# faverogian/diffusion-classifier

Hardware: AMD Instinct MI355X
Metric: images classified/sec (node), CIFAR-10 10-class x 50-step ELBO scoring (higher is better)
Workload: dtype bf16; 1 GPU; cifar10-unet-10x50; classes=10, trials=50, forwards_per_image=500, input=uniform [-1,1], parallelism=single

## Files before the change

diffusion-classifier_amd/csrc/conv3_halo.h:

```cpp
#pragma once
#include <stdlib.h>
#include "igemm_epilogue.h"

typedef const __attribute__((address_space(1))) void* gptr_t;
typedef __attribute__((address_space(3))) void* lptr_t;

struct HaloGeom {
  int ltw, lth, lni;
  int tiles_x, tiles_y;
  int hw, hp, HR, nxl;
  int n_img, H, W;
  float inv_hp, inv_hw;
  int mos, lmc;
  float inv_ch, inv_cw;
  int xbuf;
  int sws;
  int lpt;
};


constexpr int HALO_WST = 128 * 64;

template <int NW> struct HaloCfg {
  static constexpr int NT = NW * 64;
  static constexpr int PIX = NW * 64;
  static constexpr int NXL = NW == 4 ? 6 : 7;
  static constexpr int XBUF = NXL * NT * 16;
  static constexpr int XROWS = NXL * NT / 4;
  static constexpr int WLD = 512 / NT;
  static constexpr int WR = NW == 4 ? 3 : 4;
  static constexpr int GNOFF = 2 * XBUF + WR * HALO_WST;
  static constexpr int GNMAXC = 512;
  static constexpr int TBLOFF = GNOFF + 2 * GNMAXC * 4;
  static constexpr int LDS_MAIN = TBLOFF + 128;
  static constexpr int LDS = LDS_MAIN;
};

__device__ __forceinline__ int swz64(int row) { return (0x78 >> (((row >> 2) & 3) << 1)) & 3; }
__device__ __forceinline__ int lds64_off(int row, int chunk) { return row * 64 + ((chunk ^ swz64(row)) << 4); }


struct HaloQs {
  static constexpr bool on = true;
  int nbase, ltp, n_img, tile_in_img, wm, np, padd;
  __device__ __forceinline__ bool whole() const { return ltp >= 7; }
  __device__ __forceinline__ int parts() const { return np; }
  __device__ __forceinline__ bool operator()(int half, int& n, int& part) const {
    const int p0 = wm * 128 + half * 64;
    n = nbase + (p0 >> ltp);
    part = padd + (ltp >= 7 ? (tile_in_img << (ltp - 7)) + ((p0 & ((1 << ltp) - 1)) >> 7) : tile_in_img);
    return n < n_img;
  }
};

struct HaloLdsBias {
  static constexpr bool on = true, has_rowvec = true;
  const float* p;
  __device__ __forceinline__ void operator()(int k, float (&bs)[8], float (&)[8]) const {
    const f32x4 lo = *reinterpret_cast<const f32x4*>(p + 32 * k), hi = *reinterpret_cast<const f32x4*>(p + 32 * k + 4);
#pragma unroll
    for (int e = 0; e < 4; ++e) { bs[e] = lo[e]; bs[4 + e] = hi[e]; }
  }
};

template <int N> __device__ __forceinline__ void hwait_vmcnt() { asm volatile("s_waitcnt vmcnt(%0)" ::"n"(N) : "memory"); }

template <int V> struct IC { static constexpr int value = V; };
```

diffusion-classifier_amd/csrc/conv3_halo.hip:

```cpp
#include <stdlib.h>
#include "common.h"
#ifdef DC_STAMPS
static __device__ unsigned long long* g_stamps;
extern "C" void dc_debug_set_stamps(unsigned long long* p) { (void)hipMemcpyToSymbol(HIP_SYMBOL(g_stamps), &p, sizeof(p)); }
#define DC_STAMP(k) do { if (threadIdx.x == 0 && g_stamps) g_stamps[blockIdx.x * 8 + (k)] = __builtin_amdgcn_s_memtime(); } while (0)
static __device__ int g_halo_abl;
extern "C" void dc_debug_set_halo_abl(int v) { (void)hipMemcpyToSymbol(HIP_SYMBOL(g_halo_abl), &v, sizeof(v)); }
#define DC_HALO_ABL() __builtin_amdgcn_readfirstlane(g_halo_abl)
#else
#define DC_STAMP(k) do {} while (0)
#define DC_HALO_ABL() 0
#endif
#include "igemm_epilogue.h"
#include "epi_pn.h"

static __device__ unsigned g_pn_timeouts;
static __device__ chunk16 g_zero_page[16];
#include "conv3_halo.h"
DC_CLOCK_DECL(conv3_halo)

template <typename T, int NW, int NTAP = 9, int MODE = 0, bool STG = false, bool PN = false>
__global__ __launch_bounds__(NW * 64, 2) void conv3_halo_kernel(const IgemmArgs a, const HaloGeom g) {
  static_assert(!PN || (MODE == 1 && NW == 4 && !STG) || ((MODE == 0 || MODE == 2) && NW == 8 && STG && NTAP == 9), "producer-side GroupNorm: one-image-per-patch forms, or 8x8 / 4x4 images");
  constexpr bool PNX = PN && NW == 4, PNL = PN && NW == 8;
  static_assert(!STG || NW == 8, "staggered loop: the 8-wave kernel");
  constexpr bool XB = MODE == 1, MOS = MODE == 2;
  using Cfg = HaloCfg<NW>;
  constexpr int EPC = Elem<T>::EPC;
  constexpr int BKE = 4 * EPC;
  constexpr int TM = 8, TN = 4;
  constexpr int NT = Cfg::NT, WLD = Cfg::WLD, WR = Cfg::WR, PD = Cfg::WR - 1;
  extern __shared__ __attribute__((aligned(16))) char smem[];
  char* const Wring = smem + 2 * Cfg::XBUF;

  DC_STAMP(0);
  const int t = threadIdx.x;
  const int lane = t & 63;
  const int wave = __builtin_amdgcn_readfirstlane(t >> 6);
  const int wm = wave >> 1, wn = wave & 1;
  const int lr = lane & 15, lq = lane >> 4;
  int tile_m, tile_n;
  if constexpr (PNX) {
    constexpr int LPH = NTAP == 4 ? 2 : 0;
    const int tnr = a.tiles_n >> LPH;
    const int kq = blockIdx.x >> 3;
    const int grp = ((kq >> (g.lpt + LPH)) << 3) + (blockIdx.x & 7);
    if (grp >= g.n_img * tnr) return;
    const int smp = grp / tnr;
    const int within = kq & ((1 << (g.lpt + LPH)) - 1);
    tile_n = __builtin_amdgcn_readfirstlane((within >> g.lpt) * tnr + grp - smp * tnr);
    tile_m = __builtin_amdgcn_readfirstlane((smp << g.lpt) + (within & ((1 << g.lpt) - 1)));
    asm volatile("" : "+s"(tile_m), "+s"(tile_n));
  } else if constexpr (XB) tile_of_block_scalar(a, tile_m, tile_n);
  else tile_of_block(a, tile_m, tile_n);
  constexpr bool UP4 = NTAP == 4;
  int phase = 0;
  if (UP4) { const int tn = a.tiles_n >> 2; phase = tile_n / tn; tile_n -= phase * tn; }
  const int pa = phase >> 1, pb = phase & 1;
  const int tx = tile_m % g.tiles_x;
  const int ty = (tile_m / g.tiles_x) % g.tiles_y;
  const int ng = tile_m / (g.tiles_x * g.tiles_y);
  const int tw = 1 << g.ltw, th = 1 << g.lth;
  const int HW = g.H * g.W;
  const int HWs = a.upsample ? (g.H >> 1) * (g.W >> 1) : HW;
  const int Ctot = a.C0 + a.C1;
  const int c0chunks = a.C0 / BKE, nchunks = Ctot / BKE;

  constexpr int NXL = Cfg::NXL;
  int pp[NXL];
  const int xlx = t & 3;
  int* const tbl = reinterpret_cast<int*>(smem + Cfg::TBLOFF);
  if (t < (1 << g.lni)) {
    const int n = (ng << g.lni) + t;
    const bool vn = n < g.n_img;
    tbl[4 * t] = vn ? (a.map0 ? a.map0[n] : n) * HWs : -1;
    tbl[4 * t + 1] = (vn && a.src1) ? (a.map1 ? a.map1[n] : n) * HWs : -1;
    tbl[4 * t + 2] = (vn && a.src2) ? (a.map2 ? a.map2[n] : n) * HWs : -1;
  }
  auto piece_code = [&](int i, int* col = nullptr) -> int {
    const int hr = (i * NT + t) >> 2;
    int code = -1;
    if (col) *col = 0;
    if (i < g.nxl && hr < g.HR) {
      if constexpr (MOS) {
        const int hy = (int)(((float)hr + 0.5f) * g.inv_hw), hx = hr - hy * g.hw;
        const int cy = (int)(((float)hy + 0.5f) * g.inv_ch), ry = hy - cy * (th + 1);
        const int cx = (int)(((float)hx + 0.5f) * g.inv_cw), rx = hx - cx * (tw + 1);
        if (col) *col = hx;
        if (ry > 0 && rx > 0) code = (((cy << g.lmc) + cx) << 20) | ((ry - 1) * g.W + rx - 1);
      } else {
        const int img = (int)(((float)hr + 0.5f) * g.inv_hp), r = hr - img * g.hp;
        const int hy = (int)(((float)r + 0.5f) * g.inv_hw), hx = r - hy * g.hw;
        const int iy = ty * th + hy - 1, ix = tx * tw + hx - 1;
        if (col) *col = hx;
        if ((unsigned)iy < (unsigned)g.H && (unsigned)ix < (unsigned)g.W)
          code = (img << 20) | (a.upsample ? (iy >> 1) * (g.W >> 1) + (ix >> 1) : iy * g.W + ix);
      }
    }
    return code;
  };
  constexpr bool SWP = !STG;
#pragma unroll
  for (int i = 0; i < NXL; ++i) {
    int col;
    pp[i] = piece_code(i, &col);
    if constexpr (SWP) { if (pp[i] >= 0) pp[i] |= ((col >> g.sws) & 1) << 30; }
  }
  auto sw_of = [&](int pk) -> int { if constexpr (SWP) return (pk >> 30) & 1; else return 0; };
  constexpr int PKMASK = SWP ? 0x3FFFFFFF : -1;
  float* const brv = reinterpret_cast<float*>(smem + Cfg::GNOFF);
  constexpr bool STAGE_BRV = XB;
  if (STAGE_BRV && t < 128) {
    const int c = tile_n * 128 + t;
    float v = 0.f;
    if (c < a.Cout) {
      if (a.bias) v = a.bias[c];
      if (a.rowvec) v += a.rowvec[(size_t)(a.rowvec_map ? a.rowvec_map[ng] : ng) * a.rowvec_ld + c];
    }
    brv[t] = v;
  }
  if constexpr (PNX) {
    if (t >= 128 && t < 256) {
      const int c = tile_n * 128 + t - 128;
      brv[t] = a.pn_gamma[c];
      brv[t + 128] = a.pn_beta[c];
    }
  }
  __syncthreads();
  const char* zero = reinterpret_cast<const char*>(g_zero_page);
  constexpr bool XROW = STG && !XB;
  auto retarget = [&](int which) {
#pragma unroll
    for (int i = 0; i < NXL; ++i) {
      const int code = piece_code(i);
      int row = -1;
      if (code >= 0) {
        const int b = tbl[4 * (code >> 20) + which];
        if (b >= 0) row = b + (code & 0xFFFFF);
      }
      pp[i] = row;
    }
  };
  if constexpr (XROW) retarget(0);

  const T* xb0 = nullptr; const T* xb1 = nullptr; const T* xb2 = nullptr;
  int wvoff = 0, ldb0 = 0, ldb1 = 0, ldb2 = 0;
  if (XB) {
    ldb0 = a.ld0 * (int)sizeof(T); ldb1 = a.ld1 * (int)sizeof(T); ldb2 = a.ld2 * (int)sizeof(T);
    asm volatile("" : "+s"(ldb0), "+s"(ldb1), "+s"(ldb2));
    const int n = ng;
    const int s0 = __builtin_amdgcn_readfirstlane(a.map0 ? a.map0[n] : n);
    xb0 = reinterpret_cast<const T*>(a.src0) + (size_t)s0 * HWs * a.ld0;
    if (a.src1) { const int s1 = __builtin_amdgcn_readfirstlane(a.map1 ? a.map1[n] : n); xb1 = reinterpret_cast<const T*>(a.src1) + (size_t)s1 * HWs * a.ld1; }
    if (a.src2) { const int s2 = __builtin_amdgcn_readfirstlane(a.map2 ? a.map2[n] : n); xb2 = reinterpret_cast<const T*>(a.src2) + (size_t)s2 * HWs * a.ld2; }
  }
  if (XB || STG) {
    const int wrow0 = t >> 2;
    wvoff = (epi_wrow(wrow0, false) * a.Ktot + ((t & 3) ^ swz64(wrow0)) * EPC) * (int)sizeof(T);
  }
  auto rsrc_of = [](const void* base) { return __builtin_amdgcn_make_buffer_rsrc(const_cast<void*>(base), 0, 0x7fffffff, 0x00020000); };

  auto issue_x = [&](int cc, int i0 = 0, int i1 = 64) {
    const int which = cc >= nchunks ? 2 : (cc >= c0chunks ? 1 : 0);
    if constexpr (XB) {
      int ldb = ldb0, cb = cc;
      const T* xb = xb0;
      if (cc >= nchunks) { ldb = ldb2; cb = cc - nchunks; xb = xb2; }
      else if (cc >= c0chunks) { ldb = ldb1; cb = cc - c0chunks; xb = xb1; }
      const int cofs = cb * 64 + xlx * 16;
      const __amdgpu_buffer_rsrc_t rs = rsrc_of(xb);
      char* xs = smem + (cc & 1) * Cfg::XBUF + wave * 1024;
#pragma unroll
      for (int i = 0; i < NXL; ++i) {
        if (i < i0 || i >= i1) continue;
        int pk = pp[i];
        asm volatile("" : "+v"(pk));
        const int voff = pk < 0 ? -1 : (pk & PKMASK) * ldb + (cofs ^ (sw_of(pk) << 5));
        __builtin_amdgcn_raw_ptr_buffer_load_lds(rs, (lptr_t)(xs + i * (NT * 16)), 16, voff, 0, 0, 0);
      }
      return;
    } else {
    const T* src = reinterpret_cast<const T*>(which == 2 ? a.src2 : (which == 1 ? a.src1 : a.src0));
    const int ld = which == 2 ? a.ld2 : (which == 1 ? a.ld1 : a.ld0);
    const int coff = (which == 2 ? cc - nchunks : (which == 1 ? cc - c0chunks : cc)) * BKE + xlx * EPC;
    char* xs = smem + (cc & 1) * Cfg::XBUF + wave * 1024;
#pragma unroll
    for (int i = 0; i < NXL; ++i) {
      if (i < i0 || i >= i1) continue;
      int pk = pp[i];
      asm volatile("" : "+v"(pk));
      int rowi;
      if constexpr (XROW) rowi = pk;
      else {
        const int base = pk < 0 ? -1 : tbl[4 * ((pk & PKMASK) >> 20) + which];
        rowi = base < 0 ? -1 : base + (pk & 0xFFFFF);
      }
      const size_t e = (size_t)(rowi < 0 ? 0 : rowi) * ld + (coff ^ (sw_of(pk) << 1) * EPC);
      const char* gp = rowi < 0 ? zero : reinterpret_cast<const char*>(src + e);
      __builtin_amdgcn_global_load_lds((gptr_t)gp, (lptr_t)(xs + i * (NT * 16)), 16, 0, 0);
    }
    }
  };
  const int wtile0 = ((UP4 ? phase * (a.tiles_n >> 2) : 0) + tile_n) * 128 * a.Ktot;
  auto issue_w = [&](int cc, int tap, int slot) {
    if constexpr (XB || STG) {
      const int so = (wtile0 + tap * Ctot + cc * BKE) * (int)sizeof(T);
      const __amdgpu_buffer_rsrc_t wrs = rsrc_of(a.W);
#pragma unroll
      for (int i = 0; i < WLD; ++i)
        __builtin_amdgcn_raw_ptr_buffer_load_lds(wrs, (lptr_t)(Wring + slot * HALO_WST + i * (NT * 16) + wave * 1024), 16, wvoff,
                                                 __builtin_amdgcn_readfirstlane(so + i * 64 * a.Ktot * (int)sizeof(T)), 0, 0);
    } else {
      const T* wb = reinterpret_cast<const T*>(a.W) + (size_t)wtile0 + (size_t)tap * Ctot + (size_t)cc * BKE;
      int tt = t;
      asm volatile("" : "+v"(tt));
#pragma unroll
      for (int i = 0; i < WLD; ++i) {
        const int row = (i * NT + tt) >> 2;
        const int wro = epi_wrow(row, false) * a.Ktot + ((tt & 3) ^ swz64(row)) * EPC;
        __builtin_amdgcn_global_load_lds((gptr_t) reinterpret_cast<const char*>(wb + wro),
                                         (lptr_t)(Wring + slot * HALO_WST + i * (NT * 16) + wave * 1024), 16, 0, 0);
      }
    }
  };

  auto issue_w2 = [&](int e, int slot) {
    int tt = t;
    asm volatile("" : "+v"(tt));
#pragma unroll
    for (int i = 0; i < WLD; ++i) {
      const int row = (i * NT + tt) >> 2;
      const T* wp = reinterpret_cast<const T*>(a.W2) + (size_t)(tile_n * 128 + epi_wrow(row, false)) * a.C2 + ((tt & 3) ^ swz64(row)) * EPC + e * BKE;
      __builtin_amdgcn_global_load_lds((gptr_t) reinterpret_cast<const char*>(wp),
                                       (lptr_t)(Wring + slot * HALO_WST + i * (NT * 16) + wave * 1024), 16, 0, 0);
    }
  };
  const int nx = a.src2 ? a.C2 / BKE : 0;

  constexpr int NV = 3;
  int xlv[NV];
  {
    const int xx = lr & ((tw < 16 ? tw : 16) - 1);
    const int rowpart = ((lr >> g.ltw) * g.hw + (lr & (tw - 1))) * 64;
#pragma unroll
    for (int k = 0; k < NV; ++k) xlv[k] = rowpart + ((lq ^ (SWP ? (((xx + k + (UP4 ? pb : 0)) >> g.sws) & 1) << 1 : 0)) << 4);
  }
  int joff[TM];
#pragma unroll
  for (int j = 0; j < TM; ++j) {
    const int p = wm * 128 + j * 16;
    const int img = p >> (g.ltw + g.lth), py = (p >> g.ltw) & (th - 1), px = p & (tw - 1);
    const int o = MOS ? ((img >> g.lmc) * (th + 1) + py) * g.hw + (img & ((1 << g.lmc) - 1)) * (tw + 1) + px : img * g.hp + py * g.hw + px;
    joff[j] = __builtin_amdgcn_readfirstlane(o * 64);
  }
  const int woff0 = lds64_off(wn * 64 + lr, lq);

  f32x4 acc[TN][TM];
#pragma unroll
  for (int i = 0; i < TN; ++i)
#pragma unroll
    for (int j = 0; j < TM; ++j) acc[i][j] = f32x4{0.f, 0.f, 0.f, 0.f};

  auto mma_tap = [&](const char* Wst, const char* Xb, int tapoff, auto kxc) {
    constexpr int kx = decltype(kxc)::value;
    chunk16 wf[TN];
#pragma unroll
    for (int i = 0; i < TN; ++i) wf[i] = *reinterpret_cast<const chunk16*>(Wst + woff0 + i * 1024);
#pragma unroll
    for (int h = 0; h < 2; ++h) {
      chunk16 xf[TM / 2];
#pragma unroll
      for (int j = 0; j < TM / 2; ++j) xf[j] = *reinterpret_cast<const chunk16*>(Xb + (tapoff + joff[h * (TM / 2) + j]) + xlv[MOS ? ((kx + j) & 1) : kx]);
#pragma unroll
      for (int j = 0; j < TM / 2; ++j)
#pragma unroll
        for (int i = 0; i < TN; ++i) acc[i][h * (TM / 2) + j] = Mma<T>::run(wf[i], xf[j], acc[i][h * (TM / 2) + j]);
      if (h == 0) __builtin_amdgcn_sched_barrier(0);
    }
  };

  DC_STAMP(1);
  if constexpr (STG) {
    const bool grpB = wave >= 4;
    const int abl = DC_HALO_ABL();
    int cur_which = 0;
    issue_x(0);
#pragma unroll
    for (int i = 0; i < PD; ++i) issue_w(0, i, i);
    hwait_vmcnt<0>();
    __builtin_amdgcn_s_barrier();
    if (grpB) __builtin_amdgcn_s_barrier();
    DC_CLOCK(0);
    chunk16 wf[TN], xf[TM / 2];
    const uint32_t lds0 = lds_addr_of(smem);
    uint32_t xaddr[TM];
#pragma unroll
    for (int j = 0; j < TM; ++j) xaddr[j] = lds0 + (uint32_t)(joff[j] + xlv[0]);
    const uint32_t waddr = lds_addr_of(Wring) + (uint32_t)woff0;
    for (int cc = 0; cc < nchunks; ++cc) {
      const bool side_next = cc + 1 == nchunks && nx > 0;
      const bool has_next = cc + 1 < nchunks || side_next;
      const int s0 = cc * NTAP;
      const uint32_t xbo = (uint32_t)(cc & 1) * Cfg::XBUF;
      if constexpr (XROW) {
        const int wnext = cc + 1 >= nchunks ? 2 : (cc + 1 >= c0chunks ? 1 : 0);
        if (has_next && wnext != cur_which) { retarget(wnext); cur_which = wnext; }
      }
      auto step = [&](auto tapc) {
        constexpr int tap = decltype(tapc)::value;
        constexpr int ky = UP4 ? (tap >> 1) : tap / 3, kx = UP4 ? (tap & 1) : tap - ky * 3;
        const uint32_t rowo = xbo + (uint32_t)(((ky + pa) * g.hw + pb) * 64);
        const uint32_t wso = (uint32_t)((s0 + tap) % WR) * HALO_WST;
        __builtin_amdgcn_s_barrier();
        __builtin_amdgcn_sched_barrier(0);
        if (!(abl & 2)) {
        wf[0] = ds_read16_async_off<0>(waddr + wso);
        wf[1] = ds_read16_async_off<1024>(waddr + wso);
        wf[2] = ds_read16_async_off<2048>(waddr + wso);
        wf[3] = ds_read16_async_off<3072>(waddr + wso);
#pragma unroll
        for (int j = 0; j < TM / 2; ++j) xf[j] = ds_read16_async_off<kx * 64>(xaddr[j] + rowo);
        }
        constexpr int t2 = tap + PD;
#ifndef DC_STG_W_IN_M
        if (!(abl & 4)) {
        if (t2 < NTAP) issue_w(cc, t2, (s0 + t2) % WR);
        else if (side_next) { if (t2 - NTAP < nx) issue_w2(t2 - NTAP, (s0 + t2) % WR); }
        else if (has_next) issue_w(cc + 1, t2 - NTAP, (s0 + t2) % WR);
        }
#endif
#ifdef DC_STG_WAIT_FIRST
        asm volatile("s_waitcnt lgkmcnt(0)" : "+v"(wf[0]), "+v"(wf[1]), "+v"(wf[2]), "+v"(wf[3]), "+v"(xf[0]), "+v"(xf[1]), "+v"(xf[2]), "+v"(xf[3]));
        __builtin_amdgcn_s_barrier();
#else
        __builtin_amdgcn_s_barrier();
        asm volatile("s_waitcnt lgkmcnt(0)" : "+v"(wf[0]), "+v"(wf[1]), "+v"(wf[2]), "+v"(wf[3]), "+v"(xf[0]), "+v"(xf[1]), "+v"(xf[2]), "+v"(xf[3]));
#endif
        __builtin_amdgcn_sched_barrier(0);
        if (!(abl & 1)) {
#pragma unroll
        for (int i = 0; i < TN; ++i) acc[i][0] = Mma<T>::run(wf[i], xf[0], acc[i][0]);
        }
        __builtin_amdgcn_sched_barrier(0);
#ifdef DC_STG_W_IN_M
        if (!(abl & 4)) {
        if (t2 < NTAP) issue_w(cc, t2, (s0 + t2) % WR);
        else if (side_next) { if (t2 - NTAP < nx) issue_w2(t2 - NTAP, (s0 + t2) % WR); }
        else if (has_next) issue_w(cc + 1, t2 - NTAP, (s0 + t2) % WR);
        }
#endif
        __builtin_amdgcn_sched_barrier(0);
        if (!(abl & 1)) {
#pragma unroll
        for (int j = 1; j < TM / 2; ++j)
#pragma unroll
          for (int i = 0; i < TN; ++i) acc[i][j] = Mma<T>::run(wf[i], xf[j], acc[i][j]);
        }
        __builtin_amdgcn_sched_barrier(0);
        __builtin_amdgcn_s_barrier();
        __builtin_amdgcn_sched_barrier(0);
        if (!(abl & 2)) {
#pragma unroll
        for (int j = 0; j < TM / 2; ++j) xf[j] = ds_read16_async_off<kx * 64>(xaddr[TM / 2 + j] + rowo);
        }
        constexpr int XP_A = UP4 ? (tap == 1 ? NXL : 0) : (tap == 1 ? 2 : (tap >= 2 && tap <= 6 ? 1 : 0));
#ifndef DC_STG_X_IN_M
        constexpr int XP_C = UP4 ? (tap == 0 ? NXL : 0) : (tap == 0 ? 2 : (tap <= 5 ? 1 : 0));
        if (has_next && !(abl & 12)) {
          if constexpr (UP4) { if (tap == 0) issue_x(cc + 1); }
          else if constexpr (tap == 0) issue_x(cc + 1, 0, 2);
          else if constexpr (tap <= 5) issue_x(cc + 1, tap + 1, tap + 2);
        }
        constexpr int XP_B = XP_C + (UP4 ? (tap == 2 ? NXL : 0) : (tap == 2 ? 2 : (tap >= 3 && tap <= 7 ? 1 : 0)));
#else
        constexpr int XP_B = UP4 ? (tap == 2 ? NXL : 0) : (tap == 2 ? 2 : (tap >= 3 && tap <= 7 ? 1 : 0));
#endif
        if (has_next) {
          if (tap == NTAP - 1 && side_next && nx < PD) hwait_vmcnt<0>();
          else hwait_vmcnt<(PD - 1) * WLD + XP_A + XP_B>();
        } else {
          constexpr int left = NTAP - 1 - tap;
          if constexpr (left > 0) hwait_vmcnt<((left - 1) < (PD - 1) ? (left - 1) : (PD - 1)) * WLD>();
        }
#ifdef DC_STG_WAIT_FIRST
        asm volatile("s_waitcnt lgkmcnt(0)" : "+v"(xf[0]), "+v"(xf[1]), "+v"(xf[2]), "+v"(xf[3]));
        __builtin_amdgcn_s_barrier();
#else
        __builtin_amdgcn_s_barrier();
        asm volatile("s_waitcnt lgkmcnt(0)" : "+v"(xf[0]), "+v"(xf[1]), "+v"(xf[2]), "+v"(xf[3]));
#endif
        __builtin_amdgcn_sched_barrier(0);
        if (!(abl & 1)) {
#pragma unroll
        for (int i = 0; i < TN; ++i) acc[i][TM / 2] = Mma<T>::run(wf[i], xf[0], acc[i][TM / 2]);
        }
        __builtin_amdgcn_sched_barrier(0);
#ifdef DC_STG_X_IN_M
        if (has_next && !(abl & 12)) {
          if constexpr (UP4) { if (tap == 0) issue_x(cc + 1); }
          else if constexpr (tap == 0) issue_x(cc + 1, 0, 2);
          else if constexpr (tap <= 5) issue_x(cc + 1, tap + 1, tap + 2);
        }
#endif
        __builtin_amdgcn_sched_barrier(0);
        if (!(abl & 1)) {
#pragma unroll
        for (int j = 1; j < TM / 2; ++j)
#pragma unroll
          for (int i = 0; i < TN; ++i) acc[i][TM / 2 + j] = Mma<T>::run(wf[i], xf[j], acc[i][TM / 2 + j]);
        }
        __builtin_amdgcn_sched_barrier(0);
      };
      step(IC<0>{}); step(IC<1>{}); step(IC<2>{}); step(IC<3>{});
      if constexpr (NTAP == 9) { step(IC<4>{}); step(IC<5>{}); step(IC<6>{}); step(IC<7>{}); step(IC<8>{}); }
    }
    if (!grpB) __builtin_amdgcn_s_barrier();
    DC_CLOCK(1);
  } else {
  issue_x(0);
#pragma unroll
  for (int i = 0; i < PD; ++i) issue_w(0, i, i);
  constexpr int FLYL = (PD - 1) * WLD;
  DC_CLOCK(0);
  for (int cc = 0; cc < nchunks; ++cc) {
    const bool side_next = cc + 1 == nchunks && nx > 0;
    const bool has_next = cc + 1 < nchunks || side_next;
    const int s0 = cc * NTAP;
    const char* Xb = smem + (cc & 1) * Cfg::XBUF;
    auto step = [&](auto tapc) {
      constexpr int tap = decltype(tapc)::value;
      if (has_next) {
        if (tap >= 1 && tap <= PD) hwait_vmcnt<FLYL + NXL>();
        else hwait_vmcnt<FLYL>();
      } else {
        constexpr int left = NTAP - 1 - tap;
        hwait_vmcnt<(left < PD - 1 ? left : PD - 1) * WLD>();
      }
      __builtin_amdgcn_s_barrier();
      constexpr int t2 = tap + PD;
      if (t2 < NTAP) issue_w(cc, t2, (s0 + t2) % WR);
      else if (side_next) { if (t2 - NTAP < nx) issue_w2(t2 - NTAP, (s0 + t2) % WR); }
      else if (has_next) issue_w(cc + 1, t2 - NTAP, (s0 + t2) % WR);
      if (tap == 0 && has_next) issue_x(cc + 1);

      const char* Wst = Wring + ((s0 + tap) % WR) * HALO_WST;
      constexpr int ky = UP4 ? (tap >> 1) : tap / 3, kx = UP4 ? (tap & 1) : tap - ky * 3;
      const int tapoff = ((ky + pa) * g.hw + kx + pb) * 64;
      mma_tap(Wst, Xb, tapoff, IC<kx>{});
    };
    step(IC<0>{}); step(IC<1>{}); step(IC<2>{}); step(IC<3>{});
    if constexpr (NTAP == 9) { step(IC<4>{}); step(IC<5>{}); step(IC<6>{}); step(IC<7>{}); step(IC<8>{}); }
  }

  DC_CLOCK(1);
  }
  constexpr int FLY = (PD - 1) * WLD;
  {
    const int NSm = nchunks * NTAP;
    for (int e = 0; e < nx; ++e) {
      if (e == 0 && nx >= PD) hwait_vmcnt<FLY>();
      else hwait_vmcnt<0>();
      __builtin_amdgcn_s_barrier();
      if (e + PD < nx) issue_w2(e + PD, (NSm + e + PD) % WR);
      if (e + 1 < nx) issue_x(nchunks + e + 1);
      const char* Xb = smem + ((nchunks + e) & 1) * Cfg::XBUF;
      const char* Wst = Wring + ((NSm + e) % WR) * HALO_WST;
      const int tapoff = (g.hw + 1) * 64;
      mma_tap(Wst, Xb, tapoff, IC<1>{});
    }
  }

  DC_STAMP(2);
  const int nw0 = min((ng << g.lni) + ((wm * 128) >> (g.ltw + g.lth)), g.n_img - 1);
  const int nw1 = min((ng << g.lni) + ((wm * 128 + 127) >> (g.ltw + g.lth)), g.n_img - 1);
  HaloQs qsfn;
  qsfn.nbase = ng << g.lni; qsfn.ltp = g.ltw + g.lth; qsfn.n_img = g.n_img; qsfn.tile_in_img = ty * g.tiles_x + tx; qsfn.wm = wm;
  qsfn.np = HW >= 128 ? HW >> 7 : 1;
  qsfn.padd = 0;
  if (UP4) { qsfn.padd = phase * qsfn.np; qsfn.np *= 4; }
  auto rowfn = [&](int j, EpiRow& r) {
    const int p = wm * 128 + j * 16 + lr;
    int n = (ng << g.lni) + (p >> (g.ltw + g.lth));
    r.ok = n < g.n_img;
    n = r.ok ? n : g.n_img - 1;
    const int py = (p >> g.ltw) & (th - 1), px = p & (tw - 1);
    const int rem = (ty * th + py) * g.W + tx * tw + px;
    r.samp = n;
    r.o = UP4 ? n * (4 * HW) + (2 * (ty * th + py) + pa) * (2 * g.W) + 2 * (tx * tw + px) + pb : n * HW + rem;
    r.r = (a.residual && a.res_map ? a.res_map[n] : n) * HW + rem;
  };
  if constexpr (PNL && MOS) {
    epi_direct_act<T, TM, DC_ACT_NONE, false, false>(a, acc, tile_n, wn, lq, nw0, nw1, rowfn, EpiNoPre(), qsfn, EpiNoBias(), EpiPnLocal4x4());
  } else if constexpr (PNL) {
    epi_direct_act<T, TM, DC_ACT_NONE, false, true>(a, acc, tile_n, wn, lq, nw0, nw1, rowfn, EpiNoPre(), qsfn, EpiNoBias(), EpiPnLocal8x8());
  } else if constexpr (PNX) {
    PnCtx pc;
    pc.sample = ng; pc.part = (UP4 ? phase * (HW >> 7) : 0) + ((ty * g.tiles_x + tx) << 1) + wm;
    pc.parts = (HW >> 7) << (UP4 ? 2 : 0); pc.tiles = 1 << (g.lpt + (UP4 ? 2 : 0));
    pc.qpg = (a.Cout / a.pn_groups) >> 2;
    pc.cnt = a.pn_cnt + (size_t)ng * (UP4 ? a.tiles_n >> 2 : a.tiles_n) + tile_n; pc.timeouts = &g_pn_timeouts;
    pc.gam = brv + 128 + wn * 64 + lq * 8; pc.bet = brv + 256 + wn * 64 + lq * 8;
    pc.scr = reinterpret_cast<float2*>(pc.tiles > 1 ? smem + wave * 4096 : smem + wn * 256);
    pc.flag = reinterpret_cast<int*>(brv + 384);
    pc.eps = a.pn_eps; pc.silu = a.pn_silu;
    epi_halo_pn<T>(a, acc, tile_n, wn, lq, rowfn, brv + wn * 64 + lq * 8, pc);
  } else if constexpr (STAGE_BRV) {
    epi_direct_act<T, TM, DC_ACT_NONE, false, true>(a, acc, tile_n, wn, lq, nw0, nw1, rowfn, EpiNoPre(), qsfn, HaloLdsBias{brv + wn * 64 + lq * 8});
  } else {
    epi_direct_act<T, TM, DC_ACT_NONE, false, !MOS>(a, acc, tile_n, wn, lq, nw0, nw1, rowfn, EpiNoPre(), qsfn);
  }
  DC_STAMP(7);
}

struct ThinCfg {
  static constexpr int NT = 256, NXL = 6;
  static constexpr int XBUF = NXL * NT * 16;
  static constexpr int WBUF = 3 * NT * 16;
  static constexpr int TBLOFF = 2 * XBUF + 2 * WBUF;
  static constexpr int LDS = TBLOFF + 128;
  static constexpr int GNOFF = LDS, GNMAXC = 512;
  static constexpr int LDS_GN = GNOFF + 2 * GNMAXC * 4;
};

template <typename T, bool GN>
__global__ __launch_bounds__(256, 2) void conv3_thin_kernel(const IgemmArgs a, const HaloGeom g) {
  using Cfg = ThinCfg;
  constexpr int EPC = Elem<T>::EPC;
  constexpr int BKE = 4 * EPC;
  constexpr int TM = 4, NT = Cfg::NT, NXL = Cfg::NXL;
  extern __shared__ __attribute__((aligned(16))) char smem[];
  char* const Wl = smem + 2 * Cfg::XBUF;
  const int t = threadIdx.x;
  const int lane = t & 63;
  const int wave = __builtin_amdgcn_readfirstlane(t >> 6);
  const int lr = lane & 15, lq = lane >> 4;
  const int tile_m = blockIdx.x;
  const int tx = tile_m % g.tiles_x;
  const int ty = (tile_m / g.tiles_x) % g.tiles_y;
  const int ng = tile_m / (g.tiles_x * g.tiles_y);
  const int tw = 1 << g.ltw, th = 1 << g.lth;
  const int HW = g.H * g.W;
  const int Ctot = a.C0 + a.C1;
  const int c0chunks = a.C0 / BKE, nchunks = Ctot / BKE;

  int pp[NXL];
  const int xlx = t & 3;
  int* const tbl = reinterpret_cast<int*>(smem + Cfg::TBLOFF);
  if (t < (1 << g.lni)) {
    const int n = (ng << g.lni) + t;
    const bool vn = n < g.n_img;
    tbl[4 * t] = vn ? (a.map0 ? a.map0[n] : n) * HW : -1;
    tbl[4 * t + 1] = (vn && a.src1) ? (a.map1 ? a.map1[n] : n) * HW : -1;
  }
#pragma unroll
  for (int i = 0; i < NXL; ++i) {
    const int hr = (i * NT + t) >> 2;
    pp[i] = -1;
    if (i < g.nxl && hr < g.HR) {
      const int img = (int)(((float)hr + 0.5f) * g.inv_hp), r = hr - img * g.hp;
      const int hy = (int)(((float)r + 0.5f) * g.inv_hw), hx = r - hy * g.hw;
      const int iy = ty * th + hy - 1, ix = tx * tw + hx - 1;
      if ((unsigned)iy < (unsigned)g.H && (unsigned)ix < (unsigned)g.W) pp[i] = (img << 20) | (iy * g.W + ix);
    }
  }
  __syncthreads();
  const char* zero = reinterpret_cast<const char*>(g_zero_page);
  auto issue = [&](int cc) {
    const int which = cc >= c0chunks ? 1 : 0;
    const T* src = reinterpret_cast<const T*>(which ? a.src1 : a.src0);
    const int ld = which ? a.ld1 : a.ld0;
    const int coff = (which ? cc - c0chunks : cc) * BKE + xlx * EPC;
    char* xs = smem + (cc & 1) * Cfg::XBUF + wave * 1024;
#pragma unroll
    for (int i = 0; i < NXL; ++i) {
      int pk = pp[i];
      asm volatile("" : "+v"(pk));
      const int base = pk < 0 ? -1 : tbl[4 * (pk >> 20) + which];
      const size_t e = (size_t)(base < 0 ? 0 : base + (pk & 0xFFFFF)) * ld + coff;
      const char* gp = base < 0 ? zero : reinterpret_cast<const char*>(src + e);
      __builtin_amdgcn_global_load_lds((gptr_t)gp, (lptr_t)(xs + i * (NT * 16)), 16, 0, 0);
    }
    char* ws = Wl + (cc & 1) * Cfg::WBUF + wave * 1024;
#pragma unroll
    for (int i = 0; i < 3; ++i) {
      const int p = i * NT + t;
      const int tap = p >> 6, row = (p >> 2) & 15;
      const bool ok = tap < 9;
      const T* wp = reinterpret_cast<const T*>(a.W) + (size_t)row * a.Ktot + (size_t)(ok ? tap : 0) * Ctot + cc * BKE + ((p & 3) ^ swz64(row)) * EPC;
      __builtin_amdgcn_global_load_lds((gptr_t)(ok ? reinterpret_cast<const char*>(wp) : zero), (lptr_t)(ws + i * (NT * 16)), 16, 0, 0);
    }
  };
  const int xl = ((lr >> g.ltw) * g.hw + (lr & (tw - 1))) * 64 + lq * 16;
  int joff[TM];
#pragma unroll
  for (int j = 0; j < TM; ++j) {
    const int p = wave * 64 + j * 16;
    const int img = p >> (g.ltw + g.lth), py = (p >> g.ltw) & (th - 1), px = p & (tw - 1);
    joff[j] = __builtin_amdgcn_readfirstlane((img * g.hp + py * g.hw + px) * 64);
  }
  const int woff0 = lds64_off(lr, lq);
  f32x4 acc[TM];
#pragma unroll
  for (int j = 0; j < TM; ++j) acc[j] = f32x4{0.f, 0.f, 0.f, 0.f};

  float* const gnp = reinterpret_cast<float*>(smem + Cfg::GNOFF);
  if constexpr (GN) {
    if (ng < g.n_img)
      for (int c = t; c < Ctot; c += NT) {
        gnp[c] = a.gn_scale[(size_t)ng * Ctot + c];
        gnp[Ctot + c] = a.gn_shift[(size_t)ng * Ctot + c];
      }
    __builtin_amdgcn_s_waitcnt(0xC07F);
  }
  issue(0);
  for (int cc = 0; cc < nchunks; ++cc) {
    hwait_vmcnt<0>();
    __builtin_amdgcn_s_barrier();
    if (cc + 1 < nchunks) issue(cc + 1);
    if constexpr (GN) {
      const float* sc = gnp + cc * BKE + xlx * EPC;
      const float* sh = sc + Ctot;
      float scr[EPC], shr[EPC];
#pragma unroll
      for (int e = 0; e < EPC; ++e) { scr[e] = sc[e]; shr[e] = sh[e]; }
#pragma unroll
      for (int i = 0; i < NXL; ++i) {
        if (pp[i] >= 0) {
          chunk16* q = reinterpret_cast<chunk16*>(smem + (cc & 1) * Cfg::XBUF + (i * NT + t) * 16);
          float f[EPC];
          chunk_to_f<T>(*q, f);
#pragma unroll
          for (int e = 0; e < EPC; ++e) {
            float v = f[e] * scr[e] + shr[e];
            if (a.gn_silu) v = silu_t<T>(v);
            f[e] = v;
          }
          *q = f_to_chunk<T>(f);
        }
      }
      __builtin_amdgcn_s_waitcnt(0xC07F);
      __builtin_amdgcn_s_barrier();
    }
    const char* Xb = smem + (cc & 1) * Cfg::XBUF;
    const char* Wb = Wl + (cc & 1) * Cfg::WBUF;
#pragma unroll
    for (int tap = 0; tap < 9; ++tap) {
      const int ky = tap / 3, kx = tap - ky * 3;
      const int tapoff = (ky * g.hw + kx) * 64;
      const chunk16 wf = *reinterpret_cast<const chunk16*>(Wb + tap * 1024 + woff0);
#pragma unroll
      for (int j = 0; j < TM; ++j) {
        const chunk16 xf = *reinterpret_cast<const chunk16*>(Xb + (tapoff + joff[j]) + xl);
        acc[j] = Mma<T>::run(wf, xf, acc[j]);
      }
    }
  }
#pragma unroll
  for (int j = 0; j < TM; ++j) {
    const int p = wave * 64 + j * 16 + lr;
    const int n = (ng << g.lni) + (p >> (g.ltw + g.lth));
    if (n >= g.n_img) continue;
    const int py = (p >> g.ltw) & (th - 1), px = p & (tw - 1);
    const size_t o = ((size_t)n * HW + (ty * th + py) * g.W + tx * tw + px) * a.out_ld;
#pragma unroll
    for (int r = 0; r < 4; ++r) {
      const int c = lq * 4 + r;
      if (c < a.Cout) store_as(a.out, o + c, a.out_dtype, acc[j][r] + (a.bias ? a.bias[c] : 0.f));
    }
  }
}

bool dc_conv3_thin_applicable(const IgemmArgs& a, int dtype) {
  static const bool off = getenv("DCAMD_NO_THIN") != nullptr;
  if (off || a.taps != 9 || a.stride != 1 || a.upsample || a.act != DC_ACT_NONE || a.gate || a.rowvec || a.residual || a.src2) return false;
  if (a.gn_scale && a.C0 + a.C1 > ThinCfg::GNMAXC) return false;
  if (a.Cout > 16) return false;
  const int H = a.Hin, W = a.Win;
  if (H < 16 || W < 16 || (H & (H - 1)) || (W & (W - 1))) return false;
  if ((long long)a.M >= (1LL << 31)) return false;
  const int bke = 64 / dc_dtype_size(dtype);
  return a.C0 % bke == 0 && a.C1 % bke == 0;
}

static int ilog2(int v) { int l = 0; while ((1 << l) < v) ++l; return l; }

bool dc_conv3_halo_applicable(const IgemmArgs& a, int dtype) {
  if (a.taps != 9 || a.stride != 1 || a.act != DC_ACT_NONE || a.gate) return false;
  const int H = a.Hin, W = a.Win;
  static const bool no_mosaic = getenv("DCAMD_NO_MOSAIC") != nullptr;
  const bool mosaic = !no_mosaic && H == 4 && W == 4 && !a.upsample;
  if (!mosaic && (H < 8 || W < 8 || (H & (H - 1)) || (W & (W - 1)))) return false;
  if ((long long)a.M >= (1LL << 31)) return false;
  const int bke = 64 / dc_dtype_size(dtype);
  if (a.C0 % bke || a.C1 % bke) return false;
  return true;
}

template <typename T, int NW>
static int launch_halo(const IgemmArgs& a0, int n_img, hipStream_t s, bool up4 = false) {
  using Cfg = HaloCfg<NW>;
  static bool attr_done_v[2] = {false, false};
  bool& attr_done = attr_done_v[up4 ? 1 : 0];
  void (*kern)(const IgemmArgs, const HaloGeom) = up4 ? conv3_halo_kernel<T, NW, 4> : conv3_halo_kernel<T, NW>;
  if (!attr_done) {
    (void)hipFuncSetAttribute(reinterpret_cast<const void*>(kern), hipFuncAttributeMaxDynamicSharedMemorySize, Cfg::LDS);
    (void)hipFuncSetAttribute(reinterpret_cast<const void*>(conv3_halo_kernel<T, NW, 9, 1>), hipFuncAttributeMaxDynamicSharedMemorySize, Cfg::LDS);
    (void)hipFuncSetAttribute(reinterpret_cast<const void*>(conv3_halo_kernel<T, NW, 4, 1>), hipFuncAttributeMaxDynamicSharedMemorySize, Cfg::LDS);
    if constexpr (NW == 8) {
      (void)hipFuncSetAttribute(reinterpret_cast<const void*>(conv3_halo_kernel<T, NW, 9, 2>), hipFuncAttributeMaxDynamicSharedMemorySize, Cfg::LDS);
      (void)hipFuncSetAttribute(reinterpret_cast<const void*>(conv3_halo_kernel<T, NW, 4, 2>), hipFuncAttributeMaxDynamicSharedMemorySize, Cfg::LDS);
    }
    attr_done = true;
  }
  IgemmArgs a = a0;
  HaloGeom g;
  g.H = a.Hin; g.W = a.Win; g.n_img = n_img;
  const int tw = g.W < 32 ? g.W : 32;
  int th = Cfg::PIX / tw; if (th > g.H) th = g.H;
  const int ni = Cfg::PIX / (tw * th);
  g.ltw = ilog2(tw); g.lth = ilog2(th); g.lni = ilog2(ni);
  g.tiles_x = g.W / tw; g.tiles_y = g.H / th;
  g.hw = tw + 2; g.hp = (th + 2) * g.hw; g.HR = ni * g.hp;
  g.mos = 0; g.lmc = 0; g.inv_ch = g.inv_cw = 0.f;
  if (g.H < 8 || g.W < 8) {
    if (NW != 8 || tw != g.W || th != g.H || ni < 2) { dc_set_error("conv3_halo: %dx%d images need the 8-wave patch", g.H, g.W); return DC_ERR_SHAPE; }
    g.mos = 1;
    g.lmc = (g.lni + 1) / 2;
    const int cols = 1 << g.lmc, rows = ni >> g.lmc;
    g.hw = cols * (tw + 1) + 1;
    g.hp = 0;
    g.HR = (rows * (th + 1) + 1) * g.hw;
    g.inv_ch = 1.0f / (float)(th + 1); g.inv_cw = 1.0f / (float)(tw + 1);
  }
  g.inv_hp = g.hp ? 1.0f / (float)g.hp : 0.f; g.inv_hw = 1.0f / (float)g.hw;
  g.sws = (g.ltw < 4 ? g.ltw : 4) - 2;
  g.lpt = ilog2(g.tiles_x * g.tiles_y);
  {
    const long long hws = (long long)(a.upsample ? (g.H >> 1) * (g.W >> 1) : g.H * g.W);
    const long long ldmax = a.ld0 > a.ld1 ? (a.ld0 > a.ld2 ? a.ld0 : a.ld2) : (a.ld1 > a.ld2 ? a.ld1 : a.ld2);
    g.xbuf = (ni == 1 && !g.mos && hws * ldmax * (long long)sizeof(T) < (1LL << 31) &&
              (long long)a.tiles_n * 128 * a.Ktot * (long long)sizeof(T) < (1LL << 31)) ? 1 : 0;
  }
  if ((long long)a.tiles_n * 128 * a.Ktot >= (1LL << 31)) { dc_set_error("conv3_halo: weight matrix of %d x %d too large", a.tiles_n * 128, a.Ktot); return DC_ERR_SHAPE; }
  g.nxl = (g.HR * 4 + Cfg::NT - 1) / Cfg::NT;
  if (g.HR > Cfg::XROWS || g.nxl > Cfg::NXL || g.nxl < 3) { dc_set_error("conv3_halo: halo of %d rows does not fit", g.HR); return DC_ERR_SHAPE; }
  a.tiles_m = ((n_img + ni - 1) / ni) * g.tiles_x * g.tiles_y;
  const long long nblk = (long long)a.tiles_m * a.tiles_n;
  if (nblk <= 0 || nblk > 0x7fffffffLL) { dc_set_error("conv3_halo: bad grid %lld", nblk); return DC_ERR_SHAPE; }
  if (g.xbuf) kern = up4 ? conv3_halo_kernel<T, NW, 4, 1> : conv3_halo_kernel<T, NW, 9, 1>;
  bool pn_local = false;
  if (a.pn_out) {
    if constexpr (NW == 4) {
      if (!g.xbuf || ni != 1) { dc_set_error("conv3_halo: producer-side GroupNorm needs the one-image-per-patch form"); return DC_ERR_SHAPE; }
      static bool pn_attr[2] = {false, false};
      kern = up4 ? conv3_halo_kernel<T, 4, 4, 1, false, true> : conv3_halo_kernel<T, 4, 9, 1, false, true>;
      if (!pn_attr[up4 ? 1 : 0]) { (void)hipFuncSetAttribute(reinterpret_cast<const void*>(kern), hipFuncAttributeMaxDynamicSharedMemorySize, Cfg::LDS); pn_attr[up4 ? 1 : 0] = true; }
    } else {
      const bool i8 = !g.mos && !g.xbuf && g.H == 8 && g.W == 8 && ni == 8, i4 = g.mos && g.H == 4 && g.W == 4 && ni == 32;
      if (up4 || !(i8 || i4)) { dc_set_error("conv3_halo: producer-side GroupNorm on the 8-wave patch needs 8x8 or 4x4 images"); return DC_ERR_SHAPE; }
      pn_local = true;
    }
  }
  if constexpr (NW == 8) {
    if (g.mos) kern = up4 ? conv3_halo_kernel<T, NW, 4, 2> : conv3_halo_kernel<T, NW, 9, 2>;
    if (!up4 && !getenv("DCAMD_HALO_NO_STAG") && (long long)a.tiles_n * 128 * a.Ktot * (long long)sizeof(T) < (1LL << 31)) {
      const int mode = pn_local ? (g.mos ? 4 : 3) : (g.mos ? 2 : (g.xbuf ? 1 : 0));
      static bool stg_attr[5] = {false, false, false, false, false};
      switch (mode) {
        case 4: kern = conv3_halo_kernel<T, NW, 9, 2, true, true>; break;
        case 3: kern = conv3_halo_kernel<T, NW, 9, 0, true, true>; break;
        case 0: kern = conv3_halo_kernel<T, NW, 9, 0, true>; break;
        case 1: kern = conv3_halo_kernel<T, NW, 9, 1, true>; break;
        default: kern = conv3_halo_kernel<T, NW, 9, 2, true>; break;
      }
      if (!stg_attr[mode]) {
        (void)hipFuncSetAttribute(reinterpret_cast<const void*>(kern), hipFuncAttributeMaxDynamicSharedMemorySize, Cfg::LDS);
        stg_attr[mode] = true;
      }
    }
  }
  if constexpr (NW == 8) {
    if (pn_local && kern != conv3_halo_kernel<T, 8, 9, 0, true, true> && kern != conv3_halo_kernel<T, 8, 9, 2, true, true>) { dc_set_error("conv3_halo: producer-side GroupNorm on 8x8 images needs the staggered loop"); return DC_ERR_SHAPE; }
  }
  long long grid = nblk;
  if (a.pn_out && !pn_local) {
    const long long groups = (long long)n_img * (up4 ? a.tiles_n >> 2 : a.tiles_n);
    grid = ((groups + 7) / 8 * 8) << (g.lpt + (up4 ? 2 : 0));
    if (grid > 0x7fffffffLL) { dc_set_error("conv3_halo: bad grid %lld", grid); return DC_ERR_SHAPE; }
  }
  hipLaunchKernelGGL(kern, dim3((unsigned)grid), dim3(Cfg::NT), Cfg::LDS, s, a, g);
  return dc_check_launch("dc_igemm(conv3_halo)");
}

constexpr int PN_MAX_TILES = 16;
bool dc_conv3_halo_pn_ok(const IgemmArgs& a, int dtype, bool up4) {
  static const bool off = getenv("DCAMD_NO_PN") != nullptr;
  if (off || a.src1) return false;
  if (!up4 && ((a.Hin == 8 && a.Win == 8) || (a.Hin == 4 && a.Win == 4 && !getenv("DCAMD_NO_MOSAIC")))) {
    if (a.upsample || !dc_conv3_halo_applicable(a, dtype) || getenv("DCAMD_HALO_NO_STAG")) return false;
    if (a.Cout % 128 || a.pn_groups <= 0 || a.Cout % a.pn_groups) return false;
    const int cpg8 = a.Cout / a.pn_groups;
    if (cpg8 != 4 && cpg8 != 8 && cpg8 != 16 && cpg8 != 32) return false;
    return (long long)a.tiles_n * 128 * a.Ktot * dc_dtype_size(dtype) < (1LL << 31);
  }
  if (up4 ? !(a.upsample && dc_conv3_up4_applicable(a, dtype)) : (a.upsample || !dc_conv3_halo_applicable(a, dtype))) return false;
  const int H = up4 ? a.Hin >> 1 : a.Hin, W = up4 ? a.Win >> 1 : a.Win;
  if (H < 16 || W < 16 || H * W < 256 || ((H * W) / 256) * (up4 ? 4 : 1) > PN_MAX_TILES) return false;
  if (a.Cout % 128 || a.pn_groups <= 0 || a.Cout % a.pn_groups) return false;
  const int cpg = a.Cout / a.pn_groups;
  if (cpg != 4 && cpg != 8 && cpg != 16 && cpg != 32) return false;
  const long long es = dc_dtype_size(dtype);
  const long long ldmax = a.ld0 > a.ld2 ? a.ld0 : a.ld2;
  if ((long long)H * W * ldmax * es >= (1LL << 31)) return false;
  if ((long long)a.tiles_n * 128 * a.Ktot * es >= (1LL << 31)) return false;
  return true;
}

unsigned dc_conv3_halo_pn_timeouts() {
  unsigned v = 0, z = 0;
  if (hipMemcpyFromSymbol(&v, HIP_SYMBOL(g_pn_timeouts), sizeof(v)) != hipSuccess) return ~0u;
  if (v) (void)hipMemcpyToSymbol(HIP_SYMBOL(g_pn_timeouts), &z, sizeof(z));
  return v;
}

bool dc_conv3_up4_applicable(const IgemmArgs& a, int dtype) {
  if (a.taps != 9 || a.stride != 1 || !a.upsample || a.act != DC_ACT_NONE || a.gate || a.gn_scale || a.src2 || a.residual) return false;
  IgemmArgs lo = a;
  lo.upsample = 0; lo.Hin = a.Hin >> 1; lo.Win = a.Win >> 1;
  return dc_conv3_halo_applicable(lo, dtype);
}

int dc_conv3_up4_launch(const IgemmArgs& a0, int dtype, int n_img, hipStream_t s) {
  IgemmArgs a = a0;
  a.upsample = 0; a.Hin = a0.Hin >> 1; a.Win = a0.Win >> 1;
  a.Ktot = 4 * (a.C0 + a.C1);
  a.tiles_n = 4 * a0.tiles_n;
  a.n_fast = 0;
  const int nw = (a.Hin <= 8 || a.Win <= 8) ? 8 : 4;
  if (nw == 8) {
    if (dtype == DC_BF16) return launch_halo<__bf16, 8>(a, n_img, s, true);
    if (dtype == DC_F16) return launch_halo<_Float16, 8>(a, n_img, s, true);
    return launch_halo<float, 8>(a, n_img, s, true);
  }
  if (dtype == DC_BF16) return launch_halo<__bf16, 4>(a, n_img, s, true);
  if (dtype == DC_F16) return launch_halo<_Float16, 4>(a, n_img, s, true);
  return launch_halo<float, 4>(a, n_img, s, true);
}

int dc_conv3_halo_launch(const IgemmArgs& a, int dtype, int n_img, hipStream_t s) {
  const int nw = (a.Hin <= 8 || a.Win <= 8) ? 8 : 4;
  if (nw == 8) {
    if (dtype == DC_BF16) return launch_halo<__bf16, 8>(a, n_img, s);
    if (dtype == DC_F16) return launch_halo<_Float16, 8>(a, n_img, s);
    return launch_halo<float, 8>(a, n_img, s);
  }
  if (dtype == DC_BF16) return launch_halo<__bf16, 4>(a, n_img, s);
  if (dtype == DC_F16) return launch_halo<_Float16, 4>(a, n_img, s);
  return launch_halo<float, 4>(a, n_img, s);
}

template <typename T>
static int launch_thin(const IgemmArgs& a0, int n_img, hipStream_t s) {
  static bool attr_done = false;
  const bool gn = a0.gn_scale != nullptr;
  void (*kern)(const IgemmArgs, const HaloGeom) = gn ? conv3_thin_kernel<T, true> : conv3_thin_kernel<T, false>;
  const int lds = gn ? ThinCfg::LDS_GN : ThinCfg::LDS;
  if (!attr_done) {
    (void)hipFuncSetAttribute(reinterpret_cast<const void*>(conv3_thin_kernel<T, false>), hipFuncAttributeMaxDynamicSharedMemorySize, ThinCfg::LDS);
    (void)hipFuncSetAttribute(reinterpret_cast<const void*>(conv3_thin_kernel<T, true>), hipFuncAttributeMaxDynamicSharedMemorySize, ThinCfg::LDS_GN);
    attr_done = true;
  }
  IgemmArgs a = a0;
  HaloGeom g;
  g.H = a.Hin; g.W = a.Win; g.n_img = n_img;
  const int tw = g.W < 32 ? g.W : 32;
  int th = 256 / tw; if (th > g.H) th = g.H;
  const int ni = 256 / (tw * th);
  g.ltw = ilog2(tw); g.lth = ilog2(th); g.lni = ilog2(ni);
  g.tiles_x = g.W / tw; g.tiles_y = g.H / th;
  g.hw = tw + 2; g.hp = (th + 2) * g.hw; g.HR = ni * g.hp;
  g.mos = 0; g.lmc = 0; g.inv_ch = g.inv_cw = 0.f; g.xbuf = 0; g.sws = 0;
  g.inv_hp = 1.0f / (float)g.hp; g.inv_hw = 1.0f / (float)g.hw;
  g.nxl = (g.HR * 4 + ThinCfg::NT - 1) / ThinCfg::NT;
  if (g.nxl > ThinCfg::NXL) { dc_set_error("conv3_thin: halo of %d rows does not fit", g.HR); return DC_ERR_SHAPE; }
  const long long nblk = (long long)((n_img + ni - 1) / ni) * g.tiles_x * g.tiles_y;
  if (nblk <= 0 || nblk > 0x7fffffffLL) { dc_set_error("conv3_thin: bad grid %lld", nblk); return DC_ERR_SHAPE; }
  if (gn && ni != 1) { dc_set_error("conv3_thin: the fused GroupNorm needs one sample per patch"); return DC_ERR_SHAPE; }
  hipLaunchKernelGGL(kern, dim3((unsigned)nblk), dim3(ThinCfg::NT), lds, s, a, g);
  return dc_check_launch("dc_igemm(conv3_thin)");
}

int dc_conv3_thin_launch(const IgemmArgs& a, int dtype, int n_img, hipStream_t s) {
  if (dtype == DC_BF16) return launch_thin<__bf16>(a, n_img, s);
  if (dtype == DC_F16) return launch_thin<_Float16>(a, n_img, s);
  return launch_thin<float>(a, n_img, s);
}
```

Measured before the change: 224.6 images/s.

## Enable staggered loop for 4-tap upsample convs and group blocks for weight-panel reuse

Lets the 8-wave upsample (4-tap phase) halo conv use the staggered-pipeline kernel variants, which it was previously excluded from. Adds a block-to-tile mapping for the 4-tap kernel that groups the four phases and several N tiles per M tile, with the group size chosen so the combined weight panels fit in about 2 MB. The aim is better L2 reuse of weights and better load overlap. It adds grid padding to multiples of 8 with early-exit blocks and new template instantiations.

```diff
diff --git a/diffusion-classifier_amd/csrc/conv3_halo.h b/diffusion-classifier_amd/csrc/conv3_halo.h
--- a/diffusion-classifier_amd/csrc/conv3_halo.h
+++ b/diffusion-classifier_amd/csrc/conv3_halo.h
@@ -16,6 +16,7 @@
   int xbuf;
   int sws;
   int lpt;
+  int lgn;
 };
 
 
diff --git a/diffusion-classifier_amd/csrc/conv3_halo.hip b/diffusion-classifier_amd/csrc/conv3_halo.hip
--- a/diffusion-classifier_amd/csrc/conv3_halo.hip
+++ b/diffusion-classifier_amd/csrc/conv3_halo.hip
@@ -51,6 +51,19 @@
     tile_n = __builtin_amdgcn_readfirstlane((within >> g.lpt) * tnr + grp - smp * tnr);
     tile_m = __builtin_amdgcn_readfirstlane((smp << g.lpt) + (within & ((1 << g.lpt) - 1)));
     asm volatile("" : "+s"(tile_m), "+s"(tile_n));
+  } else if constexpr (NTAP == 4) {
+    const int tnr = a.tiles_n >> 2, nsub = tnr >> g.lgn;
+    const int kq = blockIdx.x >> 3;
+    const int grp = ((kq >> (g.lgn + 2)) << 3) + (blockIdx.x & 7);
+    if (grp >= a.tiles_m * nsub) return;
+    const int within = kq & ((4 << g.lgn) - 1);
+    tile_m = grp / nsub;
+    tile_n = (within >> g.lgn) * tnr + ((grp - tile_m * nsub) << g.lgn) + (within & ((1 << g.lgn) - 1));
+    if constexpr (XB) {
+      tile_m = __builtin_amdgcn_readfirstlane(tile_m);
+      tile_n = __builtin_amdgcn_readfirstlane(tile_n);
+      asm volatile("" : "+s"(tile_m), "+s"(tile_n));
+    } else asm volatile("" : "+v"(tile_m), "+v"(tile_n));
   } else if constexpr (XB) tile_of_block_scalar(a, tile_m, tile_n);
   else tile_of_block(a, tile_m, tile_n);
   constexpr bool UP4 = NTAP == 4;
@@ -763,14 +776,17 @@
   }
   if constexpr (NW == 8) {
     if (g.mos) kern = up4 ? conv3_halo_kernel<T, NW, 4, 2> : conv3_halo_kernel<T, NW, 9, 2>;
-    if (!up4 && !getenv("DCAMD_HALO_NO_STAG") && (long long)a.tiles_n * 128 * a.Ktot * (long long)sizeof(T) < (1LL << 31)) {
-      const int mode = pn_local ? (g.mos ? 4 : 3) : (g.mos ? 2 : (g.xbuf ? 1 : 0));
-      static bool stg_attr[5] = {false, false, false, false, false};
+    if (!getenv("DCAMD_HALO_NO_STAG") && (long long)a.tiles_n * 128 * a.Ktot * (long long)sizeof(T) < (1LL << 31)) {
+      const int mode = (pn_local ? (g.mos ? 4 : 3) : (g.mos ? 2 : (g.xbuf ? 1 : 0))) + (up4 ? 5 : 0);
+      static bool stg_attr[8] = {false, false, false, false, false, false, false, false};
       switch (mode) {
         case 4: kern = conv3_halo_kernel<T, NW, 9, 2, true, true>; break;
         case 3: kern = conv3_halo_kernel<T, NW, 9, 0, true, true>; break;
         case 0: kern = conv3_halo_kernel<T, NW, 9, 0, true>; break;
         case 1: kern = conv3_halo_kernel<T, NW, 9, 1, true>; break;
+        case 5: kern = conv3_halo_kernel<T, NW, 4, 0, true>; break;
+        case 6: kern = conv3_halo_kernel<T, NW, 4, 1, true>; break;
+        case 7: kern = conv3_halo_kernel<T, NW, 4, 2, true>; break;
         default: kern = conv3_halo_kernel<T, NW, 9, 2, true>; break;
       }
       if (!stg_attr[mode]) {
@@ -783,9 +799,17 @@
     if (pn_local && kern != conv3_halo_kernel<T, 8, 9, 0, true, true> && kern != conv3_halo_kernel<T, 8, 9, 2, true, true>) { dc_set_error("conv3_halo: producer-side GroupNorm on 8x8 images needs the staggered loop"); return DC_ERR_SHAPE; }
   }
   long long grid = nblk;
+  g.lgn = 0;
   if (a.pn_out && !pn_local) {
     const long long groups = (long long)n_img * (up4 ? a.tiles_n >> 2 : a.tiles_n);
     grid = ((groups + 7) / 8 * 8) << (g.lpt + (up4 ? 2 : 0));
+    if (grid > 0x7fffffffLL) { dc_set_error("conv3_halo: bad grid %lld", grid); return DC_ERR_SHAPE; }
+  } else if (up4) {
+    const int tnr = a.tiles_n >> 2;
+    const long long panel = 128LL * a.Ktot * (long long)sizeof(T);
+    while (!(tnr & ((2 << g.lgn) - 1)) && 4 * (2LL << g.lgn) * panel <= (2LL << 20)) ++g.lgn;
+    const long long groups = (long long)a.tiles_m * (tnr >> g.lgn);
+    grid = ((groups + 7) / 8 * 8) << (g.lgn + 2);
     if (grid > 0x7fffffffLL) { dc_set_error("conv3_halo: bad grid %lld", grid); return DC_ERR_SHAPE; }
   }
   hipLaunchKernelGGL(kern, dim3((unsigned)grid), dim3(Cfg::NT), Cfg::LDS, s, a, g);
```

Measured after the change: 226.3 images/s (median of 6 runs). No clear change (+0.7%).
